# MAC-VO/MAC-VO

Hardware: NVIDIA H100
Metric: stereo frames/sec @640x480 (higher is better)
Workload: dtype f32

## Files before the change

### include/macvo_b200.h

```cpp
#ifndef MACVO_B200_H
#define MACVO_B200_H

#include <stddef.h>
#include <stdint.h>

#ifdef __cplusplus
extern "C" {
#endif

#define MACVO_OK 0
#define MACVO_E_ARG (-1)
#define MACVO_E_WORKSPACE (-2)
#define MACVO_E_UNSUPPORTED (-3)
#define MACVO_E_DRIVER (-4)

const char* macvo_b200_version(void);

#define MACVO_CORR_SIMT 0
#define MACVO_CORR_TC_3XF16 1
#define MACVO_CORR_TC_1XF16 2
#define MACVO_CORR_TC_TF32 3
#define MACVO_CORR_KMAJOR_INPUT 16
size_t macvo_corr_workspace_bytes(int batch, int dim, int n, int mode);
int macvo_corr_build(const float* fmap1, const float* fmap2, float* corr, int batch, int dim, int n, int mode,
// ... 77 lines not shown
                            const double* disp_cov, int k_capacity, const int* k_dev, int min_k, const double* intr,
                            double* pose_io, const macvo_pgo_params_t* params, double* stats, void* stream);

size_t macvo_pgo_exchange_bytes(int world);
int macvo_p2p_alloc(size_t bytes, void** dev_ptr, unsigned char* ipc_handle64);
int macvo_p2p_open(const unsigned char* ipc_handle64, void** peer_ptr);
int macvo_p2p_close(void* peer_ptr);
int macvo_p2p_free(void* dev_ptr);
int macvo_pgo_solve_sharded(const double* pos_Tw, const double* kp2_uv, const double* kp2_disp, const double* uv_cov,
                            const double* disp_cov, int k_shard, const int* k_total_dev, int k_offset, int min_k,
                            const double* intr, double* pose_io, const macvo_pgo_params_t* params, double* stats,
                            void* const* exchange_bufs, int world, int rank, void* stream);

#define MACVO_PGO_ACC 55
#define MACVO_PGO_MAX_RANKS 8
int macvo_pgo_accumulate(const double* pos_Tw, const double* kp2_uv, const double* kp2_disp, const double* uv_cov,
                         const double* disp_cov, int k, const double* intr, const double* pose, double huber_delta,
                         double* acc, void* stream);

int macvo_layer_norm(const float* x, const float* weight, const float* bias, float* y, long long rows,
                     int channels, float eps, void* stream);
int macvo_add_layer_norm(const float* x, const float* resid, const float* weight, const float* bias, float* sum_out,
                         float* y, long long rows, int channels, float eps, void* stream);
int macvo_patch_embed_conv1(const float* maps, const float* weight, const float* bias, float* out,
                            long long n_maps, int h, int w, int allow_tf32, void* stream);
int macvo_add_rows_relu(float* x, const float* term, long long rows, int period, int channels, void* stream);
int macvo_small_attention(const float* q, const float* k, const float* v, float* out, int batch, int nq, int nk,
                          int heads, int head_dim, int q_broadcast, int allow_tf32, void* stream);

int macvo_small_attention_ex(const float* q, const float* k, const float* v, float* out, int batch, int nq, int nk,
                             int heads, int head_dim, int q_broadcast, int allow_tf32, int ldq, int ldk, int ldv,
                             const float* q_add, const float* k_add, int add_period, void* stream);

int macvo_latent_pool(const float* tokens, const float* ut, const float* wv, const float* bv, float* out,
                      long long n_maps, int nk, void* stream);

int macvo_gru_input(const float* mf, const float* agg, const float* gamma, float* buf0, float* buf1, float* buf2,
                    float* buf3, long long pixels, void* stream);
int macvo_gru_gates(const float* zr, const float* bias, const float* hx, float* z_out, float* rhx, long long pixels,
                    void* stream);
int macvo_gru_blend(const float* q, const float* bias, const float* z, float* hx, float* h_dense, long long pixels,
                    void* stream);
size_t macvo_rows_count(int batch, int height, int width, int vertical);
void macvo_tc_set_timeline(void* buf, int capacity);
void macvo_conv_tc_set_trace(void* buf);
int macvo_conv_tc(const void* in_rows, int in_channels, int in_dense, const void* weights, const float* bias, int n_pad,
// ... 54 lines not shown
```

### mac-vo_b200/build.py

```python
from __future__ import annotations

import hashlib
import os
import shutil
import subprocess
import sys

PKG_DIR = os.path.dirname(os.path.abspath(__file__))
CSRC = os.path.join(PKG_DIR, "csrc")
LIB_DIR = os.path.join(PKG_DIR, "lib")
LIB_PATH = os.path.join(LIB_DIR, "libmacvo_b200.so")
SOURCES = ["corr_build.cu", "corr_build_simt.cu", "corr_build_tc.cu", "corr_lookup.cu", "dense_select.cu",
           "cov2to3.cu", "pgo.cu", "nn_kernels.cu", "decoder_fused.cu", "observe.cu", "decoder_token.cu", "motion_interp.cu",
           "gru_conv_tc.cu", "conv_tc.cu", "posenet.cu"]
NVCC_FLAGS = ["-gencode", "arch=compute_90a,code=sm_90a", "-O3", "-lineinfo", "-std=c++17",
              "-Xcompiler", "-fPIC", "--use_fast_math=false"]


def _nvcc() -> str:
    for cand in (os.environ.get("NVCC"), shutil.which("nvcc"), "/usr/local/cuda/bin/nvcc"):
        if cand and os.path.exists(cand):
            return cand
    raise RuntimeError("nvcc not found (CUDA 12.9 toolkit expected at /usr/local/cuda)")


def _fingerprint() -> str:
    h = hashlib.sha256()
    for name in sorted(os.listdir(CSRC)) + ["../../include/macvo_b200.h"]:
        with open(os.path.join(CSRC, name), "rb") as f:
            h.update(name.encode())
            h.update(f.read())
    h.update(" ".join(NVCC_FLAGS).encode())
    return h.hexdigest()


def build(force: bool = False, verbose: bool = True) -> str:
    os.makedirs(LIB_DIR, exist_ok=True)
# ... 34 lines not shown
```

### mac-vo_b200/csrc/common.cuh

```cuda
#pragma once
#include <cuda_runtime.h>
#include <stdint.h>
#include "../../include/macvo_b200.h"

#define MACVO_CUDA_TRY(expr)                         \
    do {                                             \
        cudaError_t _e = (expr);                     \
        if (_e != cudaSuccess) return (int)_e;       \
    } while (0)

#define MACVO_LAUNCH_CHECK()                         \
    do {                                             \
        cudaError_t _e = cudaGetLastError();         \
        if (_e != cudaSuccess) return (int)_e;       \
    } while (0)

static inline cudaStream_t as_stream(void* s) { return reinterpret_cast<cudaStream_t>(s); }

__host__ __device__ static inline int ceil_div(int a, int b) { return (a + b - 1) / b; }

template <typename T>
__device__ __forceinline__ T warp_sum(T v) {
#pragma unroll
    for (int o = 16; o > 0; o >>= 1) v += __shfl_xor_sync(0xffffffffu, v, o);
    return v;
}
```

### mac-vo_b200/csrc/decoder_token.cu

```cuda
#include "common.cuh"
#include "rows_layout.cuh"
#include <cuda_fp16.h>

namespace {

constexpr int C = 64, CF = 81, OUTC = 160;
constexpr int W_FTE0 = 0, W_FTE2 = W_FTE0 + CF * C, W_Q = W_FTE2 + C * C, W_PROJ = W_Q + C * C,
              W_FFN0 = W_PROJ + 2 * C * C, W_FFN3 = W_FFN0 + C * C, W_END = W_FFN3 + C * C;
constexpr int V_BFTE0 = W_END, V_BFTE2 = V_BFTE0 + C, V_LN1W = V_BFTE2 + C, V_LN1B = V_LN1W + C, V_BQ = V_LN1B + C,
              V_BPROJ = V_BQ + C, V_LN2W = V_BPROJ + C, V_LN2B = V_LN2W + C, V_BFFN0 = V_LN2B + C, V_BFFN3 = V_BFFN0 + C,
              V_FREQ = V_BFFN3 + C, BLOB = V_FREQ + 16;
template <int TP> struct Lay {
    static constexpr int LD = TP + 4, NT = 4 * TP;
    static constexpr int S_X0 = BLOB, S_CAT = S_X0 + CF * LD, S_A = S_CAT + 2 * C * LD, S_END = S_A + C * LD;
    static_assert(BLOB % 4 == 0 && S_X0 % 4 == 0 && S_CAT % 4 == 0 && S_A % 4 == 0, "float4 alignment");
    static_assert(S_END * 4 <= 227 * 1024, "shared memory budget");
};

__device__ __forceinline__ float gelu_erf(float x) { return 0.5f * x * (1.f + erff(x * 0.70710678118654752440f)); }

template <int K, int LD>
__device__ __forceinline__ void gemm_tile(const float* __restrict__ WT, const float* __restrict__ X, int og, int pg,
                                          float (&acc)[4][4]) {
#pragma unroll 4
    for (int k = 0; k < K; ++k) {
        const float4 w = *reinterpret_cast<const float4*>(WT + k * C + 4 * og);
        const float4 x = *reinterpret_cast<const float4*>(X + k * LD + 4 * pg);
        acc[0][0] = fmaf(w.x, x.x, acc[0][0]); acc[0][1] = fmaf(w.x, x.y, acc[0][1]);
        acc[0][2] = fmaf(w.x, x.z, acc[0][2]); acc[0][3] = fmaf(w.x, x.w, acc[0][3]);
        acc[1][0] = fmaf(w.y, x.x, acc[1][0]); acc[1][1] = fmaf(w.y, x.y, acc[1][1]);
        acc[1][2] = fmaf(w.y, x.z, acc[1][2]); acc[1][3] = fmaf(w.y, x.w, acc[1][3]);
        acc[2][0] = fmaf(w.z, x.x, acc[2][0]); acc[2][1] = fmaf(w.z, x.y, acc[2][1]);
        acc[2][2] = fmaf(w.z, x.z, acc[2][2]); acc[2][3] = fmaf(w.z, x.w, acc[2][3]);
        acc[3][0] = fmaf(w.w, x.x, acc[3][0]); acc[3][1] = fmaf(w.w, x.y, acc[3][1]);
        acc[3][2] = fmaf(w.w, x.z, acc[3][2]); acc[3][3] = fmaf(w.w, x.w, acc[3][3]);
    }
}

enum Epi { EPI_BIAS, EPI_GELU, EPI_RESID };

template <int EPI, int LD>
__device__ __forceinline__ void store_tile(float* __restrict__ Y, const float* __restrict__ bias,
// ... 253 lines not shown
```

### mac-vo_b200/csrc/wgmma_ops.cuh

```cuda
#pragma once
#include <stdint.h>

template <int N> struct Wgmma;

template <> struct Wgmma<32> {
    static constexpr int R = 16;
    __device__ __forceinline__ static void f16(float (&d)[16], uint64_t da, uint64_t db, uint32_t acc) {
        asm volatile(
            "{\n\t.reg .pred p;\n\t"
            "setp.ne.b32 p, %18, 0;\n\t"
            "wgmma.mma_async.sync.aligned.m64n32k16.f32.f16.f16 "
            "{%0, %1, %2, %3, %4, %5, %6, %7, %8, %9, %10, %11, %12, %13, %14, %15}, "
            "%16, %17, p, 1, 1, 0, 0;\n\t}"
            : "+f"(d[0]), "+f"(d[1]), "+f"(d[2]), "+f"(d[3]), "+f"(d[4]), "+f"(d[5]), "+f"(d[6]), "+f"(d[7]), "+f"(d[8]), "+f"(d[9]), "+f"(d[10]), "+f"(d[11]), "+f"(d[12]), "+f"(d[13]), "+f"(d[14]), "+f"(d[15])
            : "l"(da), "l"(db), "r"(acc));
    }
};

template <> struct Wgmma<64> {
    static constexpr int R = 32;
    __device__ __forceinline__ static void f16(float (&d)[32], uint64_t da, uint64_t db, uint32_t acc) {
        asm volatile(
            "{\n\t.reg .pred p;\n\t"
            "setp.ne.b32 p, %34, 0;\n\t"
            "wgmma.mma_async.sync.aligned.m64n64k16.f32.f16.f16 "
            "{%0, %1, %2, %3, %4, %5, %6, %7, %8, %9, %10, %11, %12, %13, %14, %15, %16, %17, %18, %19, %20, %21, %22, %23, %24, %25, %26, %27, %28, %29, %30, %31}, "
            "%32, %33, p, 1, 1, 0, 0;\n\t}"
            : "+f"(d[0]), "+f"(d[1]), "+f"(d[2]), "+f"(d[3]), "+f"(d[4]), "+f"(d[5]), "+f"(d[6]), "+f"(d[7]), "+f"(d[8]), "+f"(d[9]), "+f"(d[10]), "+f"(d[11]), "+f"(d[12]), "+f"(d[13]), "+f"(d[14]), "+f"(d[15]), "+f"(d[16]), "+f"(d[17]), "+f"(d[18]), "+f"(d[19]), "+f"(d[20]), "+f"(d[21]), "+f"(d[22]), "+f"(d[23]), "+f"(d[24]), "+f"(d[25]), "+f"(d[26]), "+f"(d[27]), "+f"(d[28]), "+f"(d[29]), "+f"(d[30]), "+f"(d[31])
            : "l"(da), "l"(db), "r"(acc));
    }
};

template <> struct Wgmma<96> {
    static constexpr int R = 48;
    __device__ __forceinline__ static void f16(float (&d)[48], uint64_t da, uint64_t db, uint32_t acc) {
        asm volatile(
            "{\n\t.reg .pred p;\n\t"
            "setp.ne.b32 p, %50, 0;\n\t"
            "wgmma.mma_async.sync.aligned.m64n96k16.f32.f16.f16 "
            "{%0, %1, %2, %3, %4, %5, %6, %7, %8, %9, %10, %11, %12, %13, %14, %15, %16, %17, %18, %19, %20, %21, %22, %23, %24, %25, %26, %27, %28, %29, %30, %31, %32, %33, %34, %35, %36, %37, %38, %39, %40, %41, %42, %43, %44, %45, %46, %47}, "
            "%48, %49, p, 1, 1, 0, 0;\n\t}"
            : "+f"(d[0]), "+f"(d[1]), "+f"(d[2]), "+f"(d[3]), "+f"(d[4]), "+f"(d[5]), "+f"(d[6]), "+f"(d[7]), "+f"(d[8]), "+f"(d[9]), "+f"(d[10]), "+f"(d[11]), "+f"(d[12]), "+f"(d[13]), "+f"(d[14]), "+f"(d[15]), "+f"(d[16]), "+f"(d[17]), "+f"(d[18]), "+f"(d[19]), "+f"(d[20]), "+f"(d[21]), "+f"(d[22]), "+f"(d[23]), "+f"(d[24]), "+f"(d[25]), "+f"(d[26]), "+f"(d[27]), "+f"(d[28]), "+f"(d[29]), "+f"(d[30]), "+f"(d[31]), "+f"(d[32]), "+f"(d[33]), "+f"(d[34]), "+f"(d[35]), "+f"(d[36]), "+f"(d[37]), "+f"(d[38]), "+f"(d[39]), "+f"(d[40]), "+f"(d[41]), "+f"(d[42]), "+f"(d[43]), "+f"(d[44]), "+f"(d[45]), "+f"(d[46]), "+f"(d[47])
            : "l"(da), "l"(db), "r"(acc));
    }
};

template <> struct Wgmma<128> {
    static constexpr int R = 64;
    __device__ __forceinline__ static void f16(float (&d)[64], uint64_t da, uint64_t db, uint32_t acc) {
        asm volatile(
// ... 76 lines not shown
```

### mac-vo_b200/flowformer_cov.py

```python
from __future__ import annotations

import math
import os
import zlib
from typing import Callable

import torch
import torch.nn.functional as F

Tensor = torch.Tensor

LATENT_TOKENS = 8
LATENT_DIM = 128
QUERY_DIM = 64
COST_INPUT_DIM = 64
VERT_C_DIM = 64
ENCODER_DEPTH = 3


def _svt_spec(prefix: str) -> list[tuple[str, tuple[int, ...], str]]:
    out: list[tuple[str, tuple[int, ...], str]] = []
    dims, heads, srs, patch, cin = (128, 256), (4, 8), (8, 4), (4, 2), (3, 128)
    for s, (C, sr, ps, ci) in enumerate(zip(dims, srs, patch, cin)):
        p = f"{prefix}.svt."
# ... 146 lines not shown
    ay = xy[..., -1:] * freq
    return torch.cat([torch.sin(ax), torch.cos(ax), torch.sin(ay), torch.cos(ay)], dim=-1)


def _f32(x: Tensor) -> Tensor:
    return x if x.dtype == torch.float64 else x.float()


def _sdpa(q: Tensor, k: Tensor, v: Tensor) -> Tensor:
    return F.scaled_dot_product_attention(q, k, v, attn_mask=None, dropout_p=0.0, is_causal=False)


class FlowFormerCovNet:

    def __init__(self, state_dict: dict[str, Tensor], device, enc_dtype=torch.float32, dec_dtype=torch.float32,
                 decoder_depth: int = 12,
                 corr_fn: Callable[[Tensor, Tensor], Tensor] | None = None,
                 lookup_fn: Callable[[Tensor, Tensor], Tensor] | None = None):
        self.device = torch.device(device)
        self.enc_dtype, self.dec_dtype, self.depth = enc_dtype, dec_dtype, decoder_depth
        self.gru_tensor_cores = os.environ.get("MACVO_B200_GRU_TC", "1") != "0"
        self.conv_tensor_cores = os.environ.get("MACVO_B200_CONV_TC", "1") != "0"
        self.gru_split_units = os.environ.get("MACVO_B200_GRU_SPLIT", "1") != "0"
        self._ops = None
        self._fused_conv_relu = True
        if corr_fn is None or lookup_fn is None or self.device.type == "cuda":
            from . import ops
            corr_fn = corr_fn or ops.corr_build
            lookup_fn = lookup_fn or ops.corr_lookup
            self._ops = ops if self.device.type == "cuda" else None
        self.corr_fn, self.lookup_fn = corr_fn, lookup_fn
        self.load_state_dict(state_dict)
        self._cache: dict = {}
        self.taps: dict | None = None

    def _tap(self, name: str, t: Tensor) -> None:
        if self.taps is not None:
            self.taps.setdefault(name, []).append(t.detach().clone())

    def load_state_dict(self, ckpt: dict[str, Tensor]) -> None:
        ckpt = {(k[7:] if k.startswith("module.") else k): v for k, v in ckpt.items()}
        W: dict[str, Tensor] = {}
        missing = []
        for key, shape, _ in param_spec():
            if key not in ckpt:
                missing.append(key)
# ... 68 lines not shown
        kh = k.reshape(B, J, heads, d).permute(0, 2, 1, 3)
        vh = v.reshape(B, J, heads, d).permute(0, 2, 1, 3)
        if I * J <= 4096:
            a = (torch.matmul(qh, kh.transpose(-1, -2)) * (d ** -0.5)).softmax(dim=-1)
            o = torch.matmul(a, vh)
        else:
            o = _sdpa(qh, kh, vh)
        return o.permute(0, 2, 1, 3).reshape(B, I, C)

    def _memo(self, key, fn):
        if key not in self._cache:
            self._cache[key] = fn()
        return self._cache[key]

    def svt(self, x: Tensor, prefix: str) -> Tensor:
        B = x.shape[0]
        for s, (heads, sr, ps) in enumerate(((4, 8, 4), (8, 4, 2))):
            p = f"{prefix}.svt."
            x = self._conv(x, p + f"patch_embeds.{s}.proj", stride=ps)
            C, H, W = x.shape[1:]
            x = self._ln(x.flatten(2).transpose(1, 2), p + f"patch_embeds.{s}.norm")
            b0, b1 = p + f"blocks.{s}.0.", p + f"blocks.{s}.1."
            x, xn = self._add_ln(x, self._svt_local_attn(self._ln(x, b0 + "norm1", 1e-6), (H, W), b0 + "attn.", heads), b0 + "norm2", 1e-6)
            x = x + self._mlp(xn, b0 + "mlp.")
            t = x.transpose(1, 2).reshape(B, C, H, W)
            t = self._conv(t, p + f"pos_block.{s}.proj.0", padding=1, groups=C) + t
            x = t.flatten(2).transpose(1, 2)
            x, xn = self._add_ln(x, self._svt_global_attn(self._ln(x, b1 + "norm1", 1e-6), (H, W), b1 + "attn.", heads, sr), b1 + "norm2", 1e-6)
            x = x + self._mlp(xn, b1 + "mlp.")
            x = x.reshape(B, H, W, C).permute(0, 3, 1, 2)
        return x

    def _mlp(self, x: Tensor, p: str) -> Tensor:
        return self._lin(F.gelu(self._lin(x, p + "fc1")), p + "fc2")

    @staticmethod
    def _to_windows(x: Tensor, ws: int) -> tuple[Tensor, tuple[int, int, int, int]]:
        B, H, W, C = x.shape
        pr, pb = (ws - W % ws) % ws, (ws - H % ws) % ws
        x = F.pad(x, (0, 0, 0, pr, 0, pb))
        nh, nw = (H + pb) // ws, (W + pr) // ws
        x = x.reshape(B, nh, ws, nw, ws, C).transpose(2, 3).reshape(B * nh * nw, ws * ws, C)
        return x, (B, nh, nw, C)

    @staticmethod
    def _from_windows(x: Tensor, meta: tuple[int, int, int, int], ws: int, H: int, W: int) -> Tensor:
        B, nh, nw, C = meta
        x = x.reshape(B, nh, nw, ws, ws, C).transpose(2, 3).reshape(B, nh * ws, nw * ws, C)
        return x[:, :H, :W, :].reshape(B, H * W, C)

    def _svt_local_attn(self, x: Tensor, size, p: str, heads: int, ws: int = 7) -> Tensor:
        B, N, C = x.shape
        H, W = size
        xw, meta = self._to_windows(x.view(B, H, W, C), ws)
        wq, bq = self.W[p + "qkv.weight"], self.W[p + "qkv.bias"]
        q, k, v = (F.linear(xw, wq[i * C:(i + 1) * C], bq[i * C:(i + 1) * C]) for i in range(3))
        o = self._attn(q, k, v, heads)
# ... 29 lines not shown
                     self.W[p + "proj.4.weight"], None if native else self.W[p + "proj.4.bias"], stride=2, padding=2)
        h, w = x.shape[2:]

        w0, b0 = self.W[p + "ffn_with_coord.0.weight"], self.W[p + "ffn_with_coord.0.bias"]

        def coord_term():
            xy = coords_grid(1, h, w, x.device, x.dtype) * 8 + 4
            enc = sine_embed(xy.view(1, 2, -1).permute(0, 2, 1), COST_INPUT_DIM)
            term = F.linear(enc, w0[:, COST_INPUT_DIM:, 0, 0], b0)
            if native:
                term = term + F.linear(self.W[p + "proj.4.bias"], w0[:, :COST_INPUT_DIM, 0, 0])
            return term.contiguous()
        term = self._memo(("pe", h, w, x.dtype, x.device, native), coord_term)
        t = x.permute(0, 2, 3, 1).reshape(M, h * w, COST_INPUT_DIM)
        t = F.linear(t, w0[:, :COST_INPUT_DIM, 0, 0])
        t = self._ops.add_rows_relu_(t, term[0]) if native else F.relu(t + term)
        t = F.linear(t, self.W[p + "ffn_with_coord.2.weight"][:, :, 0, 0], self.W[p + "ffn_with_coord.2.bias"])
        return self._ln(t, p + "norm")

    def _latent_layer(self, x: Tensor, p: str) -> Tensor:
        y = self._ln(x, p + "norm1")
        a = self._attn(self._lin(y, p + "q"), self._lin(y, p + "k"), self._lin(y, p + "v"), 8)
        x, xn = self._add_ln(x, self._lin(a, p + "proj"), p + "norm2")
        return x + self._lin(F.gelu(self._lin(xn, p + "ffn.0")), p + "ffn.3")

    def _context_tokens(self, context: Tensor, p: str, reps: int) -> Tensor:
        b, _, H, W = context.shape
        c = self._lin(context.flatten(2).permute(0, 2, 1), p + "context_proj").view(b, H, W, -1)
        return c.repeat(reps, 1, 1, 1)

    def _vert_local_attn_native(self, x: Tensor, size, context: Tensor, p: str, ws: int, heads: int) -> Tensor:
        Bt, N, C = x.shape
        H, W = size
        b = context.shape[0]
        wq, wk = self.W[p + "q.weight"], self.W[p + "k.weight"]
        enc = self._memo(("win", ws, C + VERT_C_DIM, x.dtype, x.device), lambda: sine_embed(
            coords_grid(1, ws, ws, x.device, x.dtype).view(1, 2, -1).permute(0, 2, 1), C + VERT_C_DIM))
        cproj = self._lin(context.flatten(2).permute(0, 2, 1), p + "context_proj").view(b, H, W, -1)
        cw, meta = self._to_windows(cproj, ws)
        w_qk_c = torch.cat([wq[:, C:], wk[:, C:]], 0)
        w_qk = torch.cat([wq, wk], 0)
        b_qk = torch.cat([self.W[p + "q.bias"], self.W[p + "k.bias"]], 0)
        terms = F.linear(cw, w_qk_c) + F.linear(enc, w_qk, b_qk)
        q_add, k_add = terms[..., :C].contiguous(), terms[..., C:].contiguous()
        w_x = self._memo(("vloc_w", p), lambda: torch.cat([wq[:, :C], wk[:, :C], self.W[p + "v.weight"]], 0).contiguous())
        b_x = self._memo(("vloc_b", p), lambda: torch.cat([torch.zeros(2 * C, device=x.device, dtype=x.dtype), self.W[p + "v.bias"]], 0))
        xw, meta = self._to_windows(x.view(Bt, H, W, C), ws)
# ... 49 lines not shown
        H, W = size
        ctx = self._context_tokens(context, p, Bt // context.shape[0])
        xg = x.view(Bt, H, W, C)
        qk = torch.cat([xg, ctx], dim=-1)
        pr, pb = (sr - W % sr) % sr, (sr - H % sr) % sr
        xg, qk = F.pad(xg, (0, 0, 0, pr, 0, pb)), F.pad(qk, (0, 0, 0, pr, 0, pb))
        Hp, Wp = H + pb, W + pr
        Cq = C + VERT_C_DIM
        enc_full = self._memo(("full", Hp, Wp, Cq, x.dtype, x.device), lambda: sine_embed(
            coords_grid(1, Hp, Wp, x.device, x.dtype).view(1, 2, -1).permute(0, 2, 1), Cq))
        q = self._lin(qk.reshape(Bt, Hp * Wp, Cq) + enc_full, p + "q")
        v_in = self._conv(xg.permute(0, 3, 1, 2), p + "sr_value", stride=sr).reshape(Bt, C, -1).permute(0, 2, 1)
        k_in = self._conv(qk.permute(0, 3, 1, 2), p + "sr_key", stride=sr).reshape(Bt, C, -1).permute(0, 2, 1)
        v_in, k_in = self._ln(v_in, p + "norm"), self._ln(k_in, p + "norm")
        enc_sub = self._memo(("sub", Hp // sr, Wp // sr, sr, C, x.dtype, x.device), lambda: sine_embed(
            coords_grid(1, Hp // sr, Wp // sr, x.device, x.dtype).view(1, 2, -1).permute(0, 2, 1) * sr, C))
        o = self._attn(q, self._lin(k_in + enc_sub, p + "k"), self._lin(v_in, p + "v"), heads)
        o = o.view(Bt, Hp, Wp, C)[:, :H, :W, :].reshape(Bt, N, C)
        return self._lin(o, p + "proj")

    def _vert_block(self, x: Tensor, size, context: Tensor, p: str, local: bool) -> Tensor:
        attn = self._vert_local_attn if local else self._vert_global_attn
        x, xn = self._add_ln(x, attn(self._ln(x, p + "norm1"), size, context, p + "attn."), p + "norm2")
        return x + self._mlp(xn, p + "mlp.")

    def cost_perceiver(self, cost_volume: Tensor, context: Tensor) -> tuple[Tensor, Tensor]:
        c = "memory_encoder.cost_perceiver_encoder."
        B, heads, H1, W1, H2, W2 = cost_volume.shape
        assert heads == 1
        cost_maps = cost_volume.view(B * H1 * W1, 1, H2, W2)
        tokens = self.patch_embed(cost_maps)
        p = c + "input_layer."
        lat = self.W[c + "latent_tokens"]
        M = tokens.shape[0]
        q = self._lin(self._ln(lat, p + "norm1"), p + "q")
        if self._native(tokens) and torch.backends.cuda.matmul.allow_tf32 and LATENT_DIM == 128 and LATENT_TOKENS == 8:
            a = self._ops.latent_pool(tokens, q[0], self.W[p + "k.weight"], self.W[p + "v.weight"], self.W[p + "v.bias"])
        else:
            a = self._attn(q, self._lin(tokens, p + "k"), self._lin(tokens, p + "v"), 8)
        x = lat + self._lin(a, p + "proj")
        x = x + self._lin(F.gelu(self._lin(self._ln(x, p + "norm2"), p + "ffn.0")), p + "ffn.3")
        short_cut = x
        N = H1 * W1
        self._join_context()
        for i in range(ENCODER_DEPTH):
            x = self._latent_layer(x, c + f"encoder_layers.{i}.")
            x = x.view(B, N, LATENT_TOKENS, -1).permute(0, 2, 1, 3).reshape(B * LATENT_TOKENS, N, -1)
            v_ = c + f"vertical_encoder_layers.{i}."
            x = self._vert_block(x, (H1, W1), context, v_ + "local_block.", True)
            x = self._vert_block(x, (H1, W1), context, v_ + "global_block.", False)
            x = x.view(B, LATENT_TOKENS, N, -1).permute(0, 2, 1, 3).reshape(B * N, LATENT_TOKENS, -1)
        return x + short_cut, cost_maps

    def memory_encoder(self, img1: Tensor, img2: Tensor, context: Tensor, shared: tuple[int, int] | None = None) -> tuple[Tensor, Tensor]:
        B = img1.shape[0]
        if shared is None:
            feats = self.svt(torch.cat([img1, img2], dim=0), "memory_encoder.feat_encoder")
            feats = self._conv(feats, "memory_encoder.channel_convertor")
            f1, f2 = feats[:B], feats[B:]
        else:
            i, j = shared
            if not (0 <= i < B and 0 <= j < B):
                raise ValueError(f"shared={shared}: image indices must lie in [0, {B})")
            keep = [k for k in range(B) if k != j]
# ... 304 lines not shown
```

### mac-vo_b200/ops.py

```python
from __future__ import annotations

import ctypes as C
import os
import threading

import torch

from .build import LIB_PATH

Tensor = torch.Tensor

CORR_SIMT, CORR_TC_3XF16, CORR_TC_1XF16, CORR_TC_TF32 = 0, 1, 2, 3
CORR_MODE_NAMES = {0: "simt", 1: "tc3", 2: "tc1", 3: "tf32"}
CORR_KMAJOR_INPUT = 16
PGO_ACC = 55

_lib = None
_lock = threading.Lock()
LAUNCHES = [0]


class MacvoB200Error(RuntimeError):
    pass

# ... 35 lines not shown
                        + [C.c_void_p] * 2),
    "macvo_pgo_solve_graph": (C.c_int, [C.c_int] + [C.c_void_p] * 8 + [C.c_int] + [C.c_void_p] * 2 + [C.POINTER(_PgoParams)]
                              + [C.c_void_p] * 2),
    "macvo_pgo_solve_counted": (C.c_int, [C.c_void_p] * 5 + [C.c_int, C.c_void_p, C.c_int] + [C.c_void_p] * 2
                                + [C.POINTER(_PgoParams)] + [C.c_void_p] * 2),
    "macvo_motion_interpolate_workspace_bytes": (C.c_size_t, [C.c_int]),
    "macvo_motion_interpolate": (C.c_int, [C.c_void_p, C.c_void_p, C.c_int, C.c_void_p, C.c_void_p, C.c_size_t, C.c_void_p]),
    "macvo_cov_sanity_filter": (C.c_int, [C.c_void_p] * 2 + [C.c_int] + [C.c_void_p] * 2),
    "macvo_observe_workspace_bytes": (C.c_size_t, [C.c_int]),
    "macvo_observe_packed_doubles": (C.c_size_t, [C.c_int]),
    "macvo_observe_pack": (C.c_int, [C.c_void_p, C.c_int, C.c_int] + [C.c_void_p] * 6 + [C.c_int] * 3 + [C.c_void_p] * 2
                           + [C.c_int] + [C.c_float] * 3 + [C.c_void_p] * 6 + [C.c_size_t, C.c_void_p]),
    "macvo_pgo_exchange_bytes": (C.c_size_t, [C.c_int]),
    "macvo_p2p_alloc": (C.c_int, [C.c_size_t, C.POINTER(C.c_void_p), C.c_char_p]),
    "macvo_p2p_open": (C.c_int, [C.c_char_p, C.POINTER(C.c_void_p)]),
    "macvo_p2p_close": (C.c_int, [C.c_void_p]),
    "macvo_p2p_free": (C.c_int, [C.c_void_p]),
    "macvo_pgo_solve_sharded": (C.c_int, [C.c_void_p] * 5 + [C.c_int, C.c_void_p, C.c_int, C.c_int] + [C.c_void_p] * 2
                                + [C.POINTER(_PgoParams)] + [C.c_void_p] * 2 + [C.c_int, C.c_int, C.c_void_p]),
    "macvo_pgo_accumulate": (C.c_int, [C.c_void_p] * 5 + [C.c_int] + [C.c_void_p] * 2 + [C.c_double]
                             + [C.c_void_p] * 2),
    "macvo_layer_norm": (C.c_int, [C.c_void_p] * 4 + [C.c_longlong, C.c_int, C.c_float, C.c_void_p]),
    "macvo_add_layer_norm": (C.c_int, [C.c_void_p] * 6 + [C.c_longlong, C.c_int, C.c_float, C.c_void_p]),
    "macvo_patch_embed_conv1": (C.c_int, [C.c_void_p] * 4 + [C.c_longlong, C.c_int, C.c_int, C.c_int, C.c_void_p]),
    "macvo_add_rows_relu": (C.c_int, [C.c_void_p] * 2 + [C.c_longlong, C.c_int, C.c_int, C.c_void_p]),
    "macvo_small_attention": (C.c_int, [C.c_void_p] * 4 + [C.c_int] * 7 + [C.c_void_p]),
    "macvo_query_prep": (C.c_int, [C.c_void_p] * 6 + [C.c_int, C.c_int, C.c_float, C.c_void_p]),
    "macvo_small_attention_ex": (C.c_int, [C.c_void_p] * 4 + [C.c_int] * 10 + [C.c_void_p] * 2 + [C.c_int, C.c_void_p]),
    "macvo_latent_pool": (C.c_int, [C.c_void_p] * 5 + [C.c_longlong, C.c_int, C.c_void_p]),
    "macvo_decoder_token_blob_floats": (C.c_size_t, []),
    "macvo_decoder_token": (C.c_int, [C.c_void_p] * 6 + [C.c_int, C.c_int, C.c_float, C.c_void_p]),
    "macvo_decoder_token_rows": (C.c_int, [C.c_void_p] * 6 + [C.c_int] * 3 + [C.c_float, C.c_void_p]),
    "macvo_gru_input": (C.c_int, [C.c_void_p] * 7 + [C.c_longlong, C.c_void_p]),
    "macvo_gru_gates": (C.c_int, [C.c_void_p] * 5 + [C.c_longlong, C.c_void_p]),
    "macvo_gru_blend": (C.c_int, [C.c_void_p] * 5 + [C.c_longlong, C.c_void_p]),
    "macvo_softmax_rows_f16": (C.c_int, [C.c_void_p] * 2 + [C.c_longlong, C.c_int, C.c_void_p]),
    "macvo_convex_upsample": (C.c_int, [C.c_void_p] * 3 + [C.c_float] + [C.c_int] * 3 + [C.c_void_p]),
    "macvo_rows_count": (C.c_size_t, [C.c_int] * 4),
    "macvo_tc_set_timeline": (None, [C.c_void_p, C.c_int]),
    "macvo_conv_tc_set_trace": (None, [C.c_void_p]),
    "macvo_conv_tc": (C.c_int, [C.c_void_p, C.c_int, C.c_int, C.c_void_p, C.c_void_p] + [C.c_int] * 7
                      + [C.c_void_p] + [C.c_int] * 3 + [C.c_void_p] + [C.c_int] * 3 + [C.c_void_p]),
    "macvo_flow_im2col": (C.c_int, [C.c_void_p] * 5 + [C.c_int] * 3 + [C.c_void_p]),
    "macvo_gru_tc_operand_rows": (C.c_size_t, [C.c_int] * 4),
    "macvo_gru_tc_set_trace": (None, [C.c_void_p]),
    "macvo_gru_tc_stage": (C.c_int, [C.c_int] * 6 + [C.c_void_p] * 8),
# ... 579 lines not shown
    if c not in LAYER_NORM_CHANNELS:
        raise MacvoB200Error(f"layer_norm: channels {c} not in {LAYER_NORM_CHANNELS}")
    y = torch.empty_like(x)
    rc = load_library().macvo_layer_norm(x.data_ptr(), _dev(weight, torch.float32, "ln weight").data_ptr(),
                                         _dev(bias, torch.float32, "ln bias").data_ptr(), y.data_ptr(),
                                         x.numel() // c, c, float(eps), _stream())
    _check(rc, "macvo_layer_norm")
    LAUNCHES[0] += 1
    return y


def add_layer_norm(x: Tensor, resid: Tensor, weight: Tensor, bias: Tensor, eps: float = 1e-5) -> tuple[Tensor, Tensor]:
    x, resid = _dev(x, torch.float32, "add_layer_norm x"), _dev(resid, torch.float32, "add_layer_norm resid")
    c = x.shape[-1]
    if c not in (128, 256, 512) or x.shape != resid.shape:
        raise MacvoB200Error(f"add_layer_norm: channels {c} / shapes {tuple(x.shape)} vs {tuple(resid.shape)} unsupported")
    s, y = torch.empty_like(x), torch.empty_like(x)
    rc = load_library().macvo_add_layer_norm(x.data_ptr(), resid.data_ptr(), _dev(weight, torch.float32, "ln weight").data_ptr(),
                                             _dev(bias, torch.float32, "ln bias").data_ptr(), s.data_ptr(), y.data_ptr(),
                                             x.numel() // c, c, float(eps), _stream())
    _check(rc, "macvo_add_layer_norm")
    LAUNCHES[0] += 1
    return s, y


def patch_embed_conv1(maps: Tensor, weight: Tensor, bias: Tensor, allow_tf32: bool | None = None, s2d: bool = False) -> Tensor:
    maps = _dev(maps, torch.float32, "patch_embed maps")
    m, one, h, w = maps.shape
    if one != 1 or tuple(weight.shape) != (16, 1, 6, 6):
        raise MacvoB200Error("patch_embed_conv1: expects (M,1,H,W) maps and a (16,1,6,6) weight")
    ho, wo = (h + 7) // 8 * 4, (w + 7) // 8 * 4
    tf32 = bool(torch.backends.cudnn.allow_tf32 if allow_tf32 is None else allow_tf32)
    if s2d and not tf32:
        raise MacvoB200Error("patch_embed_conv1: the space-to-depth output exists for the TF32 tensor-core variant only")
    out = torch.empty((m, ho // 2, wo // 2, 64) if s2d else (m, ho, wo, 16), dtype=torch.float32, device=maps.device)
    rc = load_library().macvo_patch_embed_conv1(maps.data_ptr(), _dev(weight, torch.float32, "w").data_ptr(),
                                                _dev(bias, torch.float32, "b").data_ptr(), out.data_ptr(),
                                                m, h, w, int(tf32) | (2 if s2d else 0), _stream())
    _check(rc, "macvo_patch_embed_conv1")
    LAUNCHES[0] += 1
    return out.permute(0, 3, 1, 2)


def space_to_depth_filter(weight: Tensor) -> Tensor:
    o, c, kh, kw = weight.shape
    if (kh, kw) != (6, 6):
# ... 468 lines not shown
```

Before: 39.94.

## Fuse transformer MLP (fc1+GELU+fc2+residual) into one TF32 wgmma kernel

Adds a warp-specialized Hopper kernel that streams fc1/fc2 weight chunks via TMA into swizzled shared memory and runs both GEMMs with TF32 wgmma. The GELU'd hidden chunk stays in shared memory and the residual add happens in the epilogue. It is wired into the SVT, vertical, and perceiver MLP blocks when channels are 128 and TF32 matmul is allowed. The aim is to remove the hidden-activation round trip to global memory and several separate launches, at the cost of TF32 rounding of activations and weights, plus a fixed tile shape that only supports hidden sizes of 128 and 512.

Measured after the change: 42.26, median of 6. +5.8%, better.

```diff
diff --git a/include/macvo_b200.h b/include/macvo_b200.h
--- a/include/macvo_b200.h
+++ b/include/macvo_b200.h
@@ -123,6 +123,8 @@
                      int channels, float eps, void* stream);
 int macvo_add_layer_norm(const float* x, const float* resid, const float* weight, const float* bias, float* sum_out,
                          float* y, long long rows, int channels, float eps, void* stream);
+int macvo_mlp_tc(const float* xn, const float* resid, const float* w1, const float* b1, const float* w2, const float* b2,
+                 float* out, int rows, int channels, int hidden, void* stream);
 int macvo_patch_embed_conv1(const float* maps, const float* weight, const float* bias, float* out,
                             long long n_maps, int h, int w, int allow_tf32, void* stream);
 int macvo_add_rows_relu(float* x, const float* term, long long rows, int period, int channels, void* stream);
diff --git a/mac-vo_b200/build.py b/mac-vo_b200/build.py
--- a/mac-vo_b200/build.py
+++ b/mac-vo_b200/build.py
@@ -12,7 +12,7 @@
 LIB_PATH = os.path.join(LIB_DIR, "libmacvo_b200.so")
 SOURCES = ["corr_build.cu", "corr_build_simt.cu", "corr_build_tc.cu", "corr_lookup.cu", "dense_select.cu",
            "cov2to3.cu", "pgo.cu", "nn_kernels.cu", "decoder_fused.cu", "observe.cu", "decoder_token.cu", "motion_interp.cu",
-           "gru_conv_tc.cu", "conv_tc.cu", "posenet.cu"]
+           "gru_conv_tc.cu", "conv_tc.cu", "posenet.cu", "mlp_tc.cu"]
 NVCC_FLAGS = ["-gencode", "arch=compute_90a,code=sm_90a", "-O3", "-lineinfo", "-std=c++17",
               "-Xcompiler", "-fPIC", "--use_fast_math=false"]
 
diff --git a/mac-vo_b200/csrc/common.cuh b/mac-vo_b200/csrc/common.cuh
--- a/mac-vo_b200/csrc/common.cuh
+++ b/mac-vo_b200/csrc/common.cuh
@@ -19,6 +19,8 @@
 
 __host__ __device__ static inline int ceil_div(int a, int b) { return (a + b - 1) / b; }
 
+__device__ __forceinline__ static float gelu_erf(float x) { return 0.5f * x * (1.f + erff(x * 0.70710678118654752440f)); }
+
 template <typename T>
 __device__ __forceinline__ T warp_sum(T v) {
 #pragma unroll
diff --git a/mac-vo_b200/csrc/decoder_token.cu b/mac-vo_b200/csrc/decoder_token.cu
--- a/mac-vo_b200/csrc/decoder_token.cu
+++ b/mac-vo_b200/csrc/decoder_token.cu
@@ -16,8 +16,6 @@
     static_assert(BLOB % 4 == 0 && S_X0 % 4 == 0 && S_CAT % 4 == 0 && S_A % 4 == 0, "float4 alignment");
     static_assert(S_END * 4 <= 227 * 1024, "shared memory budget");
 };
-
-__device__ __forceinline__ float gelu_erf(float x) { return 0.5f * x * (1.f + erff(x * 0.70710678118654752440f)); }
 
 template <int K, int LD>
 __device__ __forceinline__ void gemm_tile(const float* __restrict__ WT, const float* __restrict__ X, int og, int pg,
diff --git a/mac-vo_b200/csrc/mlp_tc.cu b/mac-vo_b200/csrc/mlp_tc.cu
--- /dev/null
+++ b/mac-vo_b200/csrc/mlp_tc.cu
@@ -0,0 +1,201 @@
+#include "tc_common.cuh"
+
+namespace {
+
+constexpr int MLP_C = 128, MLP_ROWS = 128, MLP_CHUNK = 64;
+constexpr int XN_BYTES = MLP_ROWS * MLP_C * 4;
+constexpr int XN_SUB = MLP_ROWS * 128;
+constexpr int W1_BYTES = MLP_CHUNK * MLP_C * 4;
+constexpr int W1_SUB = MLP_CHUNK * 128;
+constexpr int W2_BYTES = MLP_C * MLP_CHUNK * 4;
+constexpr int W2_SUB = MLP_C * 128;
+constexpr int HID_WG_BYTES = 64 * MLP_CHUNK * 4;
+constexpr int HID_SUB = 64 * 128;
+constexpr int OFF_W1 = XN_BYTES, OFF_W2 = OFF_W1 + 2 * W1_BYTES, OFF_HID = OFF_W2 + 2 * W2_BYTES;
+constexpr int OFF_BAR = OFF_HID + 2 * HID_WG_BYTES;
+constexpr int MLP_SMEM = OFF_BAR + 128 + 1024;
+static_assert(MLP_SMEM <= 227 * 1024, "shared memory budget");
+
+constexpr uint32_t SW128_DESC_HI = (1024u >> 4) | (1u << 30);
+__device__ __forceinline__ uint32_t sw128_lo(uint32_t smem_addr) { return ((smem_addr & 0x3FFFFu) >> 4) | (1u << 16); }
+__device__ __forceinline__ uint64_t sw128_desc(uint32_t lo) { return ((uint64_t)SW128_DESC_HI << 32) | lo; }
+
+__device__ __forceinline__ uint32_t to_tf32(float x) {
+    uint32_t r;
+    asm("cvt.rn.tf32.f32 %0, %1;" : "=r"(r) : "f"(x));
+    return r;
+}
+
+constexpr int MLP_THREADS = TC_CONSUMER_THREADS + 128;
+
+__global__ void __launch_bounds__(MLP_THREADS, 1)
+mlp_tc_kernel(const __grid_constant__ CUtensorMap map_x, const __grid_constant__ CUtensorMap map_w1,
+              const __grid_constant__ CUtensorMap map_w2, const float* __restrict__ b1, const float* __restrict__ b2,
+              const float* __restrict__ resid, float* __restrict__ out, int m, int hd) {
+    extern __shared__ uint8_t smem_raw[];
+    uint8_t* smem = reinterpret_cast<uint8_t*>((reinterpret_cast<uintptr_t>(smem_raw) + 1023) & ~(uintptr_t)1023);
+    const uint32_t s_base = smem_u32(smem);
+    const uint32_t bar_x = s_base + OFF_BAR, bar_w1f = bar_x + 8, bar_w1e = bar_w1f + 16, bar_w2f = bar_w1e + 16,
+                   bar_w2e = bar_w2f + 16;
+    const int warp = threadIdx.x >> 5, lane = threadIdx.x & 31;
+    const int m0 = blockIdx.x * MLP_ROWS, chunks = hd / MLP_CHUNK;
+
+    if (threadIdx.x == 0) {
+        mbar_init(bar_x, 1);
+        for (int s = 0; s < 2; ++s) {
+            mbar_init(bar_w1f + 8 * s, 1); mbar_init(bar_w1e + 8 * s, 2);
+            mbar_init(bar_w2f + 8 * s, 1); mbar_init(bar_w2e + 8 * s, 2);
+        }
+        fence_barrier_init();
+        prefetch_tmap(&map_x); prefetch_tmap(&map_w1); prefetch_tmap(&map_w2);
+    }
+    __syncthreads();
+
+    if (warp >= TC_PRODUCER_WARP) {
+        asm volatile("setmaxnreg.dec.sync.aligned.u32 40;");
+        if (warp == TC_PRODUCER_WARP && elect_one()) {
+            mbar_expect_tx(bar_x, XN_BYTES);
+            for (int kc = 0; kc < 4; ++kc) tma_load_2d(s_base + kc * XN_SUB, &map_x, bar_x, 32 * kc, m0);
+            for (int j = 0; j < chunks; ++j) {
+                const int s = j & 1;
+                const uint32_t parity = ((j >> 1) & 1) ^ 1;
+                mbar_wait(bar_w1e + 8 * s, parity);
+                mbar_expect_tx(bar_w1f + 8 * s, W1_BYTES);
+                for (int kc = 0; kc < 4; ++kc)
+                    tma_load_2d(s_base + OFF_W1 + s * W1_BYTES + kc * W1_SUB, &map_w1, bar_w1f + 8 * s, 32 * kc, j * MLP_CHUNK);
+                mbar_wait(bar_w2e + 8 * s, parity);
+                mbar_expect_tx(bar_w2f + 8 * s, W2_BYTES);
+                for (int h = 0; h < 2; ++h)
+                    tma_load_2d(s_base + OFF_W2 + s * W2_BYTES + h * W2_SUB, &map_w2, bar_w2f + 8 * s, j * MLP_CHUNK + 32 * h, 0);
+            }
+        }
+        return;
+    }
+
+    asm volatile("setmaxnreg.inc.sync.aligned.u32 232;");
+    const int wg = warp >> 2;
+    const bool leader = (threadIdx.x & 127) == 0;
+    const uint32_t hid = s_base + OFF_HID + wg * HID_WG_BYTES;
+    const uint32_t xa = sw128_lo(s_base) + (wg * 64 * 128 >> 4), hid_d = sw128_lo(hid);
+    const int fr = (warp & 3) * 16 + (lane >> 2), fc = 2 * (lane & 3);
+    float acc[64], h0[32], h1[32];
+
+    auto gemm1 = [&](float (&h)[32], int j) {
+        const int s = j & 1;
+        mbar_wait(bar_w1f + 8 * s, (j >> 1) & 1);
+        uint32_t xd = xa;
+        asm volatile("" : "+r"(xd));
+        const uint32_t wb = xd - (wg * 64 * 128 >> 4) + ((OFF_W1 + s * W1_BYTES) >> 4);
+        wgmma_fence();
+#pragma unroll
+        for (int kc = 0; kc < 4; ++kc) {
+#pragma unroll
+            for (int k = 0; k < 4; ++k)
+                Wgmma<64>::tf32(h, sw128_desc(xd + (kc * XN_SUB >> 4) + 2 * k), sw128_desc(wb + (kc * W1_SUB >> 4) + 2 * k), (kc | k) != 0);
+        }
+        wgmma_commit();
+    };
+
+    auto chunk = [&](float (&h)[32], float (&hn)[32], int j) {
+        if (j + 1 < chunks) {
+            gemm1(hn, j + 1);
+            wgmma_wait<1>();
+        } else {
+            wgmma_wait<0>();
+        }
+        fence_acc(h);
+        fence_acc(acc);
+        if (leader) {
+            mbar_arrive(bar_w1e + 8 * (j & 1));
+            if (j > 0) mbar_arrive(bar_w2e + 8 * ((j - 1) & 1));
+        }
+        const float* bj = b1 + j * MLP_CHUNK;
+#pragma unroll
+        for (int i = 0; i < 32; i += 2) {
+            const int r = fr + 8 * ((i >> 1) & 1), c = 8 * (i >> 2) + fc;
+            const float2 bb = __ldg(reinterpret_cast<const float2*>(bj + c));
+            const uint32_t v0 = to_tf32(gelu_erf(h[i] + bb.x)), v1 = to_tf32(gelu_erf(h[i + 1] + bb.y));
+            const int cc = c & 31;
+            const uint32_t addr = hid + (c >> 5) * HID_SUB + r * 128 + ((((cc >> 2) ^ (r & 7))) << 4) + (cc & 3) * 4;
+            asm volatile("st.shared.v2.b32 [%0], {%1, %2};" ::"r"(addr), "r"(v0), "r"(v1) : "memory");
+        }
+        asm volatile("fence.proxy.async.shared::cta;" ::: "memory");
+        if (wg == 0) asm volatile("bar.sync 2, 128;" ::: "memory");
+        else asm volatile("bar.sync 3, 128;" ::: "memory");
+        const int s = j & 1;
+        mbar_wait(bar_w2f + 8 * s, (j >> 1) & 1);
+        uint32_t hd_ = hid_d;
+        asm volatile("" : "+r"(hd_));
+        const uint32_t wb = hd_ - ((OFF_HID + wg * HID_WG_BYTES) >> 4) + ((OFF_W2 + s * W2_BYTES) >> 4);
+        wgmma_fence();
+#pragma unroll
+        for (int hh = 0; hh < 2; ++hh) {
+#pragma unroll
+            for (int k = 0; k < 4; ++k)
+                Wgmma<128>::tf32(acc, sw128_desc(hd_ + (hh * HID_SUB >> 4) + 2 * k), sw128_desc(wb + (hh * W2_SUB >> 4) + 2 * k),
+                                 (j | hh | k) != 0);
+        }
+        wgmma_commit();
+    };
+
+    mbar_wait(bar_x, 0);
+    {
+        const int t = threadIdx.x & 127;
+#pragma unroll
+        for (int kc = 0; kc < 4; ++kc) {
+#pragma unroll
+            for (int u = 0; u < 4; ++u) {
+                const uint32_t a = s_base + kc * XN_SUB + wg * 64 * 128 + (u * 128 + t) * 16;
+                const float4 v = lds128(a);
+                asm volatile("st.shared.v4.b32 [%0], {%1, %2, %3, %4};" ::"r"(a), "r"(to_tf32(v.x)), "r"(to_tf32(v.y)),
+                             "r"(to_tf32(v.z)), "r"(to_tf32(v.w)) : "memory");
+            }
+        }
+        asm volatile("fence.proxy.async.shared::cta;" ::: "memory");
+        if (wg == 0) asm volatile("bar.sync 2, 128;" ::: "memory");
+        else asm volatile("bar.sync 3, 128;" ::: "memory");
+    }
+    gemm1(h0, 0);
+    for (int j = 0; j < chunks; j += 2) {
+        chunk(h0, h1, j);
+        chunk(h1, h0, j + 1);
+    }
+    wgmma_wait<0>();
+    fence_acc(acc);
+
+    const int row0 = m0 + wg * 64 + fr;
+#pragma unroll
+    for (int i = 0; i < 64; i += 2) {
+        const int r = row0 + 8 * ((i >> 1) & 1), c = 8 * (i >> 2) + fc;
+        if (r < m) {
+            const float2 bb = __ldg(reinterpret_cast<const float2*>(b2 + c));
+            const float2 x = __ldg(reinterpret_cast<const float2*>(resid + (long long)r * MLP_C + c));
+            *reinterpret_cast<float2*>(out + (long long)r * MLP_C + c) = make_float2(x.x + (acc[i] + bb.x), x.y + (acc[i + 1] + bb.y));
+        }
+    }
+}
+
+}
+
+int macvo_mlp_tc(const float* xn, const float* resid, const float* w1, const float* b1, const float* w2, const float* b2,
+                 float* out, int rows, int channels, int hidden, void* stream) {
+    if (!xn || !resid || !w1 || !b1 || !w2 || !b2 || !out || rows <= 0) return MACVO_E_ARG;
+    if (channels != MLP_C || (hidden != 128 && hidden != 512)) return MACVO_E_UNSUPPORTED;
+    for (const void* p : {(const void*)xn, (const void*)resid, (const void*)w1, (const void*)b1, (const void*)w2,
+                          (const void*)b2, (const void*)out})
+        if (reinterpret_cast<uintptr_t>(p) & 15) return MACVO_E_ARG;
+    CUtensorMap m_x, m_w1, m_w2;
+    bool ok = make_map_2d(&m_x, CU_TENSOR_MAP_DATA_TYPE_FLOAT32, 4, xn, MLP_C, rows, MLP_C * 4, 32, MLP_ROWS);
+    ok = ok && make_map_2d(&m_w1, CU_TENSOR_MAP_DATA_TYPE_FLOAT32, 4, w1, MLP_C, hidden, MLP_C * 4, 32, MLP_CHUNK);
+    ok = ok && make_map_2d(&m_w2, CU_TENSOR_MAP_DATA_TYPE_FLOAT32, 4, w2, hidden, MLP_C, (uint64_t)hidden * 4, 32, MLP_C);
+    if (!ok) return MACVO_E_DRIVER;
+    static bool configured = false;
+    if (!configured) {
+        MACVO_CUDA_TRY(cudaFuncSetAttribute(mlp_tc_kernel, cudaFuncAttributeMaxDynamicSharedMemorySize, MLP_SMEM));
+        configured = true;
+    }
+    mlp_tc_kernel<<<ceil_div(rows, MLP_ROWS), MLP_THREADS, MLP_SMEM, as_stream(stream)>>>(m_x, m_w1, m_w2, b1, b2, resid, out,
+                                                                                          rows, hidden);
+    MACVO_LAUNCH_CHECK();
+    return MACVO_OK;
+}
diff --git a/mac-vo_b200/csrc/wgmma_ops.cuh b/mac-vo_b200/csrc/wgmma_ops.cuh
--- a/mac-vo_b200/csrc/wgmma_ops.cuh
+++ b/mac-vo_b200/csrc/wgmma_ops.cuh
@@ -26,6 +26,16 @@
             "wgmma.mma_async.sync.aligned.m64n64k16.f32.f16.f16 "
             "{%0, %1, %2, %3, %4, %5, %6, %7, %8, %9, %10, %11, %12, %13, %14, %15, %16, %17, %18, %19, %20, %21, %22, %23, %24, %25, %26, %27, %28, %29, %30, %31}, "
             "%32, %33, p, 1, 1, 0, 0;\n\t}"
+            : "+f"(d[0]), "+f"(d[1]), "+f"(d[2]), "+f"(d[3]), "+f"(d[4]), "+f"(d[5]), "+f"(d[6]), "+f"(d[7]), "+f"(d[8]), "+f"(d[9]), "+f"(d[10]), "+f"(d[11]), "+f"(d[12]), "+f"(d[13]), "+f"(d[14]), "+f"(d[15]), "+f"(d[16]), "+f"(d[17]), "+f"(d[18]), "+f"(d[19]), "+f"(d[20]), "+f"(d[21]), "+f"(d[22]), "+f"(d[23]), "+f"(d[24]), "+f"(d[25]), "+f"(d[26]), "+f"(d[27]), "+f"(d[28]), "+f"(d[29]), "+f"(d[30]), "+f"(d[31])
+            : "l"(da), "l"(db), "r"(acc));
+    }
+    __device__ __forceinline__ static void tf32(float (&d)[32], uint64_t da, uint64_t db, uint32_t acc) {
+        asm volatile(
+            "{\n\t.reg .pred p;\n\t"
+            "setp.ne.b32 p, %34, 0;\n\t"
+            "wgmma.mma_async.sync.aligned.m64n64k8.f32.tf32.tf32 "
+            "{%0, %1, %2, %3, %4, %5, %6, %7, %8, %9, %10, %11, %12, %13, %14, %15, %16, %17, %18, %19, %20, %21, %22, %23, %24, %25, %26, %27, %28, %29, %30, %31}, "
+            "%32, %33, p, 1, 1;\n\t}"
             : "+f"(d[0]), "+f"(d[1]), "+f"(d[2]), "+f"(d[3]), "+f"(d[4]), "+f"(d[5]), "+f"(d[6]), "+f"(d[7]), "+f"(d[8]), "+f"(d[9]), "+f"(d[10]), "+f"(d[11]), "+f"(d[12]), "+f"(d[13]), "+f"(d[14]), "+f"(d[15]), "+f"(d[16]), "+f"(d[17]), "+f"(d[18]), "+f"(d[19]), "+f"(d[20]), "+f"(d[21]), "+f"(d[22]), "+f"(d[23]), "+f"(d[24]), "+f"(d[25]), "+f"(d[26]), "+f"(d[27]), "+f"(d[28]), "+f"(d[29]), "+f"(d[30]), "+f"(d[31])
             : "l"(da), "l"(db), "r"(acc));
     }
diff --git a/mac-vo_b200/flowformer_cov.py b/mac-vo_b200/flowformer_cov.py
--- a/mac-vo_b200/flowformer_cov.py
+++ b/mac-vo_b200/flowformer_cov.py
@@ -192,6 +192,7 @@
         self.gru_tensor_cores = os.environ.get("MACVO_B200_GRU_TC", "1") != "0"
         self.conv_tensor_cores = os.environ.get("MACVO_B200_CONV_TC", "1") != "0"
         self.gru_split_units = os.environ.get("MACVO_B200_GRU_SPLIT", "1") != "0"
+        self.mlp_tensor_cores = os.environ.get("MACVO_B200_MLP_TC", "1") != "0"
         self._ops = None
         self._fused_conv_relu = True
         if corr_fn is None or lookup_fn is None or self.device.type == "cuda":
@@ -306,17 +307,22 @@
             x = self._ln(x.flatten(2).transpose(1, 2), p + f"patch_embeds.{s}.norm")
             b0, b1 = p + f"blocks.{s}.0.", p + f"blocks.{s}.1."
             x, xn = self._add_ln(x, self._svt_local_attn(self._ln(x, b0 + "norm1", 1e-6), (H, W), b0 + "attn.", heads), b0 + "norm2", 1e-6)
-            x = x + self._mlp(xn, b0 + "mlp.")
+            x = self._mlp_residual(x, xn, b0 + "mlp.", "fc1", "fc2")
             t = x.transpose(1, 2).reshape(B, C, H, W)
             t = self._conv(t, p + f"pos_block.{s}.proj.0", padding=1, groups=C) + t
             x = t.flatten(2).transpose(1, 2)
             x, xn = self._add_ln(x, self._svt_global_attn(self._ln(x, b1 + "norm1", 1e-6), (H, W), b1 + "attn.", heads, sr), b1 + "norm2", 1e-6)
-            x = x + self._mlp(xn, b1 + "mlp.")
+            x = self._mlp_residual(x, xn, b1 + "mlp.", "fc1", "fc2")
             x = x.reshape(B, H, W, C).permute(0, 3, 1, 2)
         return x
 
-    def _mlp(self, x: Tensor, p: str) -> Tensor:
-        return self._lin(F.gelu(self._lin(x, p + "fc1")), p + "fc2")
+    def _mlp_residual(self, x: Tensor, xn: Tensor, p: str, fc1: str, fc2: str) -> Tensor:
+        w1 = self.W[p + fc1 + ".weight"]
+        if (self.mlp_tensor_cores and self._native(x) and torch.backends.cuda.matmul.allow_tf32 and x.shape[-1] == 128
+                and w1.shape[0] in self._ops.MLP_TC_HIDDEN and x.is_contiguous() and xn.is_contiguous()):
+            w1t, w2t = self._memo(("mlp_tc", p), lambda: (self._ops.round_tf32(w1), self._ops.round_tf32(self.W[p + fc2 + ".weight"])))
+            return self._ops.mlp_tc(xn, x, w1t, self.W[p + fc1 + ".bias"], w2t, self.W[p + fc2 + ".bias"])
+        return x + self._lin(F.gelu(self._lin(xn, p + fc1)), p + fc2)
 
     @staticmethod
     def _to_windows(x: Tensor, ws: int) -> tuple[Tensor, tuple[int, int, int, int]]:
@@ -392,7 +398,7 @@
         y = self._ln(x, p + "norm1")
         a = self._attn(self._lin(y, p + "q"), self._lin(y, p + "k"), self._lin(y, p + "v"), 8)
         x, xn = self._add_ln(x, self._lin(a, p + "proj"), p + "norm2")
-        return x + self._lin(F.gelu(self._lin(xn, p + "ffn.0")), p + "ffn.3")
+        return self._mlp_residual(x, xn, p, "ffn.0", "ffn.3")
 
     def _context_tokens(self, context: Tensor, p: str, reps: int) -> Tensor:
         b, _, H, W = context.shape
@@ -488,7 +494,7 @@
     def _vert_block(self, x: Tensor, size, context: Tensor, p: str, local: bool) -> Tensor:
         attn = self._vert_local_attn if local else self._vert_global_attn
         x, xn = self._add_ln(x, attn(self._ln(x, p + "norm1"), size, context, p + "attn."), p + "norm2")
-        return x + self._mlp(xn, p + "mlp.")
+        return self._mlp_residual(x, xn, p + "mlp.", "fc1", "fc2")
 
     def cost_perceiver(self, cost_volume: Tensor, context: Tensor) -> tuple[Tensor, Tensor]:
         c = "memory_encoder.cost_perceiver_encoder."
@@ -505,7 +511,7 @@
         else:
             a = self._attn(q, self._lin(tokens, p + "k"), self._lin(tokens, p + "v"), 8)
         x = lat + self._lin(a, p + "proj")
-        x = x + self._lin(F.gelu(self._lin(self._ln(x, p + "norm2"), p + "ffn.0")), p + "ffn.3")
+        x = self._mlp_residual(x, self._ln(x, p + "norm2"), p, "ffn.0", "ffn.3")
         short_cut = x
         N = H1 * W1
         self._join_context()
diff --git a/mac-vo_b200/ops.py b/mac-vo_b200/ops.py
--- a/mac-vo_b200/ops.py
+++ b/mac-vo_b200/ops.py
@@ -81,6 +81,7 @@
                              + [C.c_void_p] * 2),
     "macvo_layer_norm": (C.c_int, [C.c_void_p] * 4 + [C.c_longlong, C.c_int, C.c_float, C.c_void_p]),
     "macvo_add_layer_norm": (C.c_int, [C.c_void_p] * 6 + [C.c_longlong, C.c_int, C.c_float, C.c_void_p]),
+    "macvo_mlp_tc": (C.c_int, [C.c_void_p] * 7 + [C.c_int] * 3 + [C.c_void_p]),
     "macvo_patch_embed_conv1": (C.c_int, [C.c_void_p] * 4 + [C.c_longlong, C.c_int, C.c_int, C.c_int, C.c_void_p]),
     "macvo_add_rows_relu": (C.c_int, [C.c_void_p] * 2 + [C.c_longlong, C.c_int, C.c_int, C.c_void_p]),
     "macvo_small_attention": (C.c_int, [C.c_void_p] * 4 + [C.c_int] * 7 + [C.c_void_p]),
@@ -706,6 +707,31 @@
     _check(rc, "macvo_add_layer_norm")
     LAUNCHES[0] += 1
     return s, y
+
+
+MLP_TC_HIDDEN = (128, 512)
+
+
+def round_tf32(w: Tensor) -> Tensor:
+    i = w.detach().to(torch.float32).contiguous().view(torch.int32)
+    return ((i + 0xFFF + ((i >> 13) & 1)) & -0x2000).view(torch.float32)
+
+
+def mlp_tc(xn: Tensor, resid: Tensor, w1: Tensor, b1: Tensor, w2: Tensor, b2: Tensor) -> Tensor:
+    xn, resid = _dev(xn, torch.float32, "mlp_tc xn"), _dev(resid, torch.float32, "mlp_tc resid")
+    w1, w2 = _dev(w1, torch.float32, "mlp_tc w1"), _dev(w2, torch.float32, "mlp_tc w2")
+    b1, b2 = _dev(b1, torch.float32, "mlp_tc b1"), _dev(b2, torch.float32, "mlp_tc b2")
+    c, hd = xn.shape[-1], w1.shape[0]
+    if (c != 128 or hd not in MLP_TC_HIDDEN or xn.shape != resid.shape or tuple(w1.shape) != (hd, c)
+            or tuple(w2.shape) != (c, hd) or b1.numel() != hd or b2.numel() != c):
+        raise MacvoB200Error(f"mlp_tc: unsupported shapes xn {tuple(xn.shape)}, resid {tuple(resid.shape)}, "
+                             f"w1 {tuple(w1.shape)}, w2 {tuple(w2.shape)}")
+    out = torch.empty_like(resid)
+    rc = load_library().macvo_mlp_tc(xn.data_ptr(), resid.data_ptr(), w1.data_ptr(), b1.data_ptr(), w2.data_ptr(),
+                                      b2.data_ptr(), out.data_ptr(), xn.numel() // c, c, hd, _stream())
+    _check(rc, "macvo_mlp_tc")
+    LAUNCHES[0] += 1
+    return out
 
 
 def patch_embed_conv1(maps: Tensor, weight: Tensor, bias: Tensor, allow_tf32: bool | None = None, s2d: bool = False) -> Tensor:
```
